# danbider/gp-quadrature

Hardware: AMD Instinct MI355X
Metric: GP-fits/sec (fit + posterior mean at the N training points), N=1e6 d=2 SE kernel (higher is better)
Workload: dtype f64; 1 GPU; 2D squared-exponential l=0.2 var=2 sigma2=0.2, eps=1e-4, global N=1e6 synthetic (BASELINE configs[1] at the metric's N=1e6), points sharded over the GPUs; n_per_gpu=1000000, global_n=1000000, d=2, mtot=23, M=529, mean_cg_iters=68, parallelism=points sharded over 1 GPU(s), CG replicated

## Files before the change

gp-quadrature_amd/csrc/nufft.hip:

```cpp
#include <cmath>
#include <cstdlib>
#include <cstring>
#include <optional>
#include <vector>

#include "common.hpp"
#include "es_kernel.hpp"
#include "nufft_dev.hpp"
#include "nufft_plan_host.hpp"
#include "points_layout.hpp"
#include "spread_mfma.hpp"
#include "small_dft.hpp"
#include "line_fft.hpp"

namespace efgp {


struct SpreadArgs {
    const double* x;
    StrengthSrc src;
    int64_t npts;
    GridGeom g;
    const double* coef;
    int degree;
// ... 1152 lines not shown
                    const double2 v = in ? f0[(int64_t)x0 * a.nf1 + x1] : make_double2(0.0, 0.0);
                    ire[u] = __double_as_longlong(v.x);
                    iim[u] = __double_as_longlong(v.y);
                } else {
                    ire[u] = in ? g0[(int64_t)x0 * a.nf1 + x1] : 0;
                    iim[u] = (in && a.channels == 2) ? g0[cells + (int64_t)x0 * a.nf1 + x1] : 0;
                }
            }
            if (r0 == 0) __syncthreads();
#pragma unroll
            for (int u = 0; u < U; ++u) {
                const double re = FINE ? __longlong_as_double(ire[u]) : (double)ire[u] * s0;
                const double im = FINE ? __longlong_as_double(iim[u]) : (double)iim[u] * s1;
#pragma unroll
                for (int jj = 0; jj < 2; ++jj) {
                    const double2 tw = T0[idx[jj]];
                    pq[jj].x += re * tw.x;
                    pq[jj].y += re * tw.y;
                    rs[jj].x += im * tw.x;
                    rs[jj].y += im * tw.y;
                    idx[jj] += step[jj];
                    if (idx[jj] >= a.nf0) idx[jj] -= a.nf0;
                }
            }
        }
#pragma unroll
        for (int jj = 0; jj < 2; ++jj) {
            Bp[grp][2 * jj][x1] = pq[jj];
            Bp[grp][2 * jj + 1][x1] = rs[jj];
        }
    }
    __syncthreads();
    unsigned int arrived = 0u;
    if (!FINE && tid == 0) arrived = atomicAdd(a.ticket, 1u);
    for (int o = tid; o < 2 * a.nf1; o += kG2MThreads) {
        const int jj = o / a.nf1, x = o - jj * a.nf1;
        double2 u = Bp[0][2 * jj][x], v = Bp[0][2 * jj + 1][x];
#pragma unroll
        for (int g = 1; g < kGroups; ++g) {
            u.x += Bp[g][2 * jj][x].x;
            u.y += Bp[g][2 * jj][x].y;
            v.x += Bp[g][2 * jj + 1][x].x;
            v.y += Bp[g][2 * jj + 1][x].y;
        }
        Bp[0][2 * jj][x] = make_double2(u.x - v.y, u.y + v.x);
        Bp[0][2 * jj + 1][x] = make_double2(u.x + v.y, v.x - u.y);
    }
    __syncthreads();
    if (nsplit > 1) {
        double2* const mine = a.partial + ((((int64_t)b * gridDim.x + blockIdx.x) * nsplit + split) * 4) * a.nf1;
        for (int o = tid; o < 4 * a.nf1; o += kG2MThreads) mine[o] = Bp[0][o / a.nf1][o % a.nf1];
        __threadfence();
        __syncthreads();
        if (tid == 0) {
            const unsigned int t = atomicAdd(a.tile_ticket + (int64_t)b * gridDim.x + blockIdx.x, 1u);
            s_last = (t == (unsigned)nsplit - 1u) ? 1 : 0;
        }
        __syncthreads();
        const bool tile_last = s_last != 0;
        __syncthreads();
        if (!tile_last) {
            if (tid == 0) s_last = (!FINE && arrived == a.total_wgs - 1u) ? 1 : 0;
            __syncthreads();
            if (s_last) {
                for (long long i = tid; i < a.acc_words; i += kG2MThreads) a.gacc[i] = 0;
                if (tid == 0) *a.ticket = 0u;
            }
            return;
        }
        __threadfence();
        const double2* const all = a.partial + (((int64_t)b * gridDim.x + blockIdx.x) * nsplit * 4) * a.nf1;
        for (int o = tid; o < 4 * a.nf1; o += kG2MThreads) {
            double2 u = all[o];
            for (int sp = 1; sp < nsplit; ++sp) {
                const double2 v = all[(int64_t)sp * 4 * a.nf1 + o];
                u.x += v.x;
                u.y += v.y;
            }
            Bp[0][o / a.nf1][o % a.nf1] = u;
        }
        if (tid == 0) a.tile_ticket[(int64_t)b * gridDim.x + blockIdx.x] = 0u;
        __syncthreads();
    }
    const int nk1 = 2 * a.h1 + 1;
    double2* const Hq = &Bp[1][0][0];
    for (int o = tid; o < 16 * nk1; o += kG2MThreads) {
        const int qtr = o / (4 * nk1), rc = o - qtr * 4 * nk1;
        const int r = rc / nk1, c = rc - r * nk1;
        int st = (c - a.h1) % a.nf1;
        if (st < 0) st += a.nf1;
        const int xa = (a.nf1 * qtr) / 4, xe = (a.nf1 * (qtr + 1)) / 4;
        int idx = (int)(((long long)st * xa) % a.nf1);
        double sx = 0.0, sy = 0.0;
        for (int x = xa; x < xe; ++x) {
            const double2 bv = Bp[0][r][x], tw = T1[idx];
            sx += bv.x * tw.x - bv.y * tw.y;
            sy += bv.x * tw.y + bv.y * tw.x;
            idx += st;
            if (idx >= a.nf1) idx -= a.nf1;
        }
        Hq[(qtr * 4 + r) * (2 * kG2MMaxH + 2) + c] = make_double2(sx, sy);
    }
    if (tid == 0) s_last = (!FINE && arrived == a.total_wgs - 1u) ? 1 : 0;
    __syncthreads();
    if (s_last) {
        for (long long i = tid; i < a.acc_words; i += kG2MThreads) a.gacc[i] = 0;
        if (tid == 0) *a.ticket = 0u;
    }
    for (int o = tid; o < 4 * nk1; o += kG2MThreads) {
        const int r = o / nk1, c = o - r * nk1;
        double2 u = Hq[r * (2 * kG2MMaxH + 2) + c];
#pragma unroll
        for (int q = 1; q < 4; ++q) {
            const double2 v = Hq[(q * 4 + r) * (2 * kG2MMaxH + 2) + c];
            u.x += v.x;
            u.y += v.y;
        }
        Hs[r][c] = u;
    }
    __syncthreads();
    for (int o = tid; o < 4 * nk1; o += kG2MThreads) {
        const int r = o / nk1, c = o - r * nk1;
        const int j = j0 + (r >> 1);
        if (j > a.h0 || (j == 0 && (r & 1))) continue;
        const int k0 = (r & 1) ? -j : j, k1 = c - a.h1;
        const double2 H = Hs[r][c], G = Hs[r ^ 1][nk1 - 1 - c];
        int64_t t;
        double f;
        if (a.part == 0) {
            if (g2m_slot(a.ma, k0, k1, &t, &f)) a.out_a[(int64_t)b * a.ma.total + t] = make_double2(H.x * f, H.y * f);
            continue;
        }
        if (g2m_slot(a.ma, k0, k1, &t, &f)) {
            double2 r1 = make_double2(0.5 * (H.x + G.x) * f, 0.5 * (H.y - G.y) * f);
            if (a.part == 3) {
                a.out_a[(int64_t)(2 * b) * a.ma.total + t] = r1;
                if (2 * b + 1 < a.rows_limit)
                    a.out_a[(int64_t)(2 * b + 1) * a.ma.total + t] = make_double2(0.5 * (H.y + G.y) * f, 0.5 * (G.x - H.x) * f);
            } else {
                const double norm0 = a.scale ? a.scale[4] : 1.0;
                if (norm0 != 1.0) {
                    r1.x *= norm0;
                    r1.y *= norm0;
                }
                a.out_a[t] = r1;
            }
        }
        if (a.part == 4 && g2m_slot(a.mb, k0, k1, &t, &f)) a.out_b[t] = make_double2(0.5 * (H.y + G.y) * f, 0.5 * (G.x - H.x) * f);
    }
}

constexpr int kG2RThreads = 1024;
constexpr int kR2MThreads = 256;

struct G2RArgs {
    long long* gacc;
    const double2* fine;
    const double* scale;
    int channels, nf0, nf1, h0, h1;
    int part, rows_limit, sign;
    ModeGeom ma, mb;
    double2* out_a;
    double2* out_b;
    double2* cbuf;
};

template <bool FINE>
__global__ __launch_bounds__(kG2RThreads) void grid_rows_kernel(G2RArgs a) {
    extern __shared__ double2 g2r_lds[];
    const int tid = threadIdx.x, b = blockIdx.y;
    const int nf0 = a.nf0, nf1 = a.nf1, h1 = a.h1;
    const int nk1 = 2 * h1 + 1;
    const int64_t cells = (int64_t)nf0 * nf1;
    double2* const T = g2r_lds;
    double2* const Row = T + 256;
    for (int q = tid; q < nf1; q += kG2RThreads) {
        double sn, cs;
        sincospi((double)a.sign * 2.0 * (double)q / (double)nf1, &sn, &cs);
        T[q] = make_double2(cs, sn);
    }
    const int x0_lo = (int)blockIdx.x * kG2RRows;
    {
        const double s0 = FINE ? 1.0 : a.scale[1], s1 = FINE ? 1.0 : a.scale[3];
        for (int o = tid; o < kG2RRows * nf1; o += kG2RThreads) {
            const int r = o / nf1, x1 = o - r * nf1, x0 = x0_lo + r;
            double2 v = make_double2(0.0, 0.0);
            if (x0 < nf0) {
                if (FINE) {
                    v = a.fine[(int64_t)b * cells + (int64_t)x0 * nf1 + x1];
                } else {
                    long long* g = a.gacc + (int64_t)b * a.channels * cells + (int64_t)x0 * nf1 + x1;
                    const long long ire = g[0];
                    g[0] = 0;
                    long long iim = 0;
                    if (a.channels == 2) {
                        iim = g[cells];
                        g[cells] = 0;
                    }
                    v = make_double2((double)ire * s0, (double)iim * s1);
                }
            }
            Row[o] = v;
        }
    }
    __syncthreads();
    constexpr int SEG = 8;
    const int seg = tid & (SEG - 1), pair = tid >> 3;
    const int npairs = kG2RRows * (h1 + 1);
    for (int pr = pair; pr < ((npairs + 127) / 128) * 128; pr += 128) {
        const bool on = pr < npairs;
        const int r = on ? pr / (h1 + 1) : 0, k1 = on ? pr - r * (h1 + 1) : 0;
        const int xa = (nf1 * seg) / SEG, xe = (nf1 * (seg + 1)) / SEG;
        int idx = (int)(((long long)k1 * xa) % nf1);
        double P = 0.0, Q = 0.0, R = 0.0, S = 0.0;
        if (on) {
            const double2* row = Row + r * nf1;
            for (int x = xa; x < xe; ++x) {
                const double2 g = row[x], tw = T[idx];
                P = fma(g.x, tw.x, P);
                Q = fma(g.x, tw.y, Q);
                R = fma(g.y, tw.x, R);
                S = fma(g.y, tw.y, S);
                idx += k1;
                if (idx >= nf1) idx -= nf1;
            }
        }
#pragma unroll
        for (int m = 1; m < SEG; m <<= 1) {
            P += __shfl_xor(P, m, 64);
            Q += __shfl_xor(Q, m, 64);
            R += __shfl_xor(R, m, 64);
            S += __shfl_xor(S, m, 64);
        }
        const int x0 = x0_lo + r;
        if (on && seg == 0 && x0 < nf0) {
            double2* c = a.cbuf + ((int64_t)b * nf0 + x0) * nk1;
            c[h1 + k1] = make_double2(P - S, Q + R);
            if (k1 > 0) c[h1 - k1] = make_double2(P + S, R - Q);
        }
    }
}

__global__ __launch_bounds__(kR2MThreads) void rows_modes_kernel(G2RArgs a) {
    __shared__ double2 T[256], Cc[2][256], Hs[2][2 * kG2MMaxH + 2], part[2][4][2 * kG2MMaxH + 2];
    const int tid = threadIdx.x, b = blockIdx.y, k1 = (int)blockIdx.x;
    const int nf0 = a.nf0, h0 = a.h0, h1 = a.h1;
    const int nk0 = 2 * h0 + 1, nk1 = 2 * h1 + 1;
    const double2* C = a.cbuf + (int64_t)b * nf0 * nk1;
    for (int o = tid; o < 2 * nf0; o += kR2MThreads) {
        const int col = o >= nf0 ? 1 : 0, x0 = o - col * nf0;
        Cc[col][x0] = C[(int64_t)x0 * nk1 + (col ? h1 - k1 : h1 + k1)];
    }
    for (int q = tid; q < nf0; q += kR2MThreads) {
        double sn, cs;
        sincospi((double)a.sign * 2.0 * (double)q / (double)nf0, &sn, &cs);
        T[q] = make_double2(cs, sn);
    }
    __syncthreads();
    for (int o = tid; o < 8 * nk0; o += kR2MThreads) {
        const int qtr = o / (2 * nk0), rc = o - qtr * 2 * nk0;
        const int col = rc / nk0, r = rc - col * nk0;
        int st = (r - h0) % nf0;
        if (st < 0) st += nf0;
        const int xa = (nf0 * qtr) / 4, xe = (nf0 * (qtr + 1)) / 4;
        int idx = (int)(((long long)st * xa) % nf0);
        double sx = 0.0, sy = 0.0;
        for (int x = xa; x < xe; ++x) {
            const double2 cv = Cc[col][x], tw = T[idx];
            sx = fma(cv.x, tw.x, fma(-cv.y, tw.y, sx));
            sy = fma(cv.x, tw.y, fma(cv.y, tw.x, sy));
            idx += st;
            if (idx >= nf0) idx -= nf0;
        }
        part[col][qtr][r] = make_double2(sx, sy);
    }
    __syncthreads();
    for (int o = tid; o < 2 * nk0; o += kR2MThreads) {
        const int col = o / nk0, r = o - col * nk0;
        Hs[col][r] = make_double2((part[col][0][r].x + part[col][1][r].x) + (part[col][2][r].x + part[col][3][r].x),
                                  (part[col][0][r].y + part[col][1][r].y) + (part[col][2][r].y + part[col][3][r].y));
    }
    __syncthreads();
    for (int o = tid; o < 2 * nk0; o += kR2MThreads) {
        const int col = o / nk0, r = o - col * nk0;
        if (col == 1 && k1 == 0) continue;
        const int k0 = r - h0, kk1 = col ? -k1 : k1;
        const double2 H = Hs[col][r], G = Hs[k1 == 0 ? 0 : 1 - col][nk0 - 1 - r];
        int64_t t;
        double f;
        if (a.part == 0) {
            if (g2m_slot(a.ma, k0, kk1, &t, &f)) a.out_a[(int64_t)b * a.ma.total + t] = make_double2(H.x * f, H.y * f);
            continue;
        }
        if (g2m_slot(a.ma, k0, kk1, &t, &f)) {
            double2 r1 = make_double2(0.5 * (H.x + G.x) * f, 0.5 * (H.y - G.y) * f);
            if (a.part == 3) {
                a.out_a[(int64_t)(2 * b) * a.ma.total + t] = r1;
                if (2 * b + 1 < a.rows_limit)
                    a.out_a[(int64_t)(2 * b + 1) * a.ma.total + t] = make_double2(0.5 * (H.y + G.y) * f, 0.5 * (G.x - H.x) * f);
            } else {
                const double norm0 = a.scale ? a.scale[4] : 1.0;
                if (norm0 != 1.0) {
                    r1.x *= norm0;
                    r1.y *= norm0;
                }
                a.out_a[t] = r1;
            }
        }
        if (a.part == 4 && g2m_slot(a.mb, k0, kk1, &t, &f)) a.out_b[t] = make_double2(0.5 * (H.y + G.y) * f, 0.5 * (G.x - H.x) * f);
    }
}

__global__ void precorrect_kernel(const double2* __restrict__ fin, const double2* __restrict__ mul, ModeGeom m, int herm,
                                  int64_t cells, double2* __restrict__ fine) {
    const int batch = blockIdx.y;
    const double2* fb = fin + (int64_t)batch * m.total;
    double2* F = fine + (int64_t)batch * cells;
    for (int64_t c = (int64_t)blockIdx.x * blockDim.x + threadIdx.x; c < cells; c += (int64_t)gridDim.x * blockDim.x) {
        int64_t rem = c;
        int64_t ks[3] = {0, 0, 0};
        bool inside = true;
        for (int a = m.d - 1; a >= 0; --a) {
            const int64_t i = rem % m.nf[a];
            rem /= m.nf[a];
            const int64_t k = i <= (m.nf[a] - 1) / 2 ? i : i - m.nf[a];
            ks[a] = k;
            inside = inside && k >= -(m.nm[a] / 2) && k <= (m.nm[a] - 1) / 2;
        }
        double2 r = make_double2(0.0, 0.0);
        if (inside) {
            int64_t t = 0, tn = 0;
            bool has_neg = true;
            double f = 1.0;
            for (int a = 0; a < m.d; ++a) {
                const int64_t k = ks[a], kmin = -(m.nm[a] / 2), kmax = (m.nm[a] - 1) / 2;
                f *= m.fac[a][k - kmin];
                t = t * m.nm[a] + (m.modeord == 0 ? k - kmin : (k >= 0 ? k : k + m.nm[a]));
                const int64_t kn = -k;
                if (kn < kmin || kn > kmax) has_neg = false;
                tn = tn * m.nm[a] + (m.modeord == 0 ? kn - kmin : (kn >= 0 ? kn : kn + m.nm[a]));
            }
            double2 v = fb[t];
            if (mul) v = make_double2(v.x * mul[t].x - v.y * mul[t].y, v.x * mul[t].y + v.y * mul[t].x);
            if (herm && has_neg) {
                double2 u = fb[tn];
                if (mul) u = make_double2(u.x * mul[tn].x - u.y * mul[tn].y, u.x * mul[tn].y + u.y * mul[tn].x);
                v = make_double2(0.5 * (v.x + u.x), 0.5 * (v.y - u.y));
            }
            r = make_double2(v.x * f, v.y * f);
        }
        F[c] = r;
    }
}

struct InterpArgs {
    const double* x;
    int64_t npts;
    GridGeom g;
    const double* coef;
    int degree;
    const double2* fine;
    void* out;
    const int* order;
    const double* image;
};

template <int D, int W, bool CPLX, bool USE_LDS>
__global__ __launch_bounds__(USE_LDS ? kInterpThreads : kInterpThreadsGlobal) void interp_kernel(InterpArgs a) {
    constexpr int kThr = USE_LDS ? kInterpThreads : kInterpThreadsGlobal;
    extern __shared__ double lds[];
    const int batch = blockIdx.y;
    const int64_t cells = a.g.cells;
    const double2* F = a.fine + (int64_t)batch * cells;
    if (USE_LDS) {
        if (CPLX) {
            double2* l2 = reinterpret_cast<double2*>(lds);
            for (int64_t i = threadIdx.x; i < cells; i += kThr) l2[i] = F[i];
        } else {
            for (int64_t i = threadIdx.x; i < cells; i += kThr) lds[i] = F[i].x;
        }
        __syncthreads();
    }
    const int nf0 = (int)a.g.nf[0], nf1 = (int)a.g.nf[1], nf2 = (int)a.g.nf[2];
    auto load = [&](int64_t i, double& re, double& im) {
        if (USE_LDS) {
            if (CPLX) {
                double2 v = reinterpret_cast<const double2*>(lds)[i];
                re = v.x;
                im = v.y;
            } else {
                re = lds[i];
                im = 0.0;
            }
        } else {
            if (CPLX) {
                double2 v = F[i];
                re = v.x;
                im = v.y;
            } else {
                re = F[i].x;
                im = 0.0;
            }
        }
    };
    for (int64_t n = (int64_t)blockIdx.x * kThr + threadIdx.x; n < a.npts;
         n += (int64_t)gridDim.x * kThr) {
        double v0[W], v1[W], v2[W];
        int f0 = 0, f1 = 0, f2 = 0;
        {
            double Xw[3] = {0.0, 0.0, 0.0};
            Xw[0] = fold(a.g.scale[0] * (a.x[n * D + 0] - a.g.xcen[0]), (double)nf0);
            if (D > 1) Xw[1] = fold(a.g.scale[1] * (a.x[n * D + 1] - a.g.xcen[1]), (double)nf1);
            if (D > 2) Xw[2] = fold(a.g.scale[2] * (a.x[n * D + 2] - a.g.xcen[2]), (double)nf2);
            window_eval<D, W>(a.coef, a.degree, Xw, nf0, nf1, nf2, f0, f1, f2, v0, v1, v2);
        }
        double sre = 0.0, sim = 0.0;
        if (D == 1) {
#pragma unroll
            for (int j = 0; j < W; ++j) {
                double re, im;
                load(wrap(f0 + j, nf0), re, im);
                sre = fma(v0[j], re, sre);
                if (CPLX) sim = fma(v0[j], im, sim);
            }
        } else if (D == 2) {
#pragma unroll
            for (int j0 = 0; j0 < W; ++j0) {
                const int row = wrap(f0 + j0, nf0) * nf1;
                double rre = 0.0, rim = 0.0;
#pragma unroll
                for (int j1 = 0; j1 < W; ++j1) {
                    double re, im;
                    load(row + wrap(f1 + j1, nf1), re, im);
                    rre = fma(v1[j1], re, rre);
                    if (CPLX) rim = fma(v1[j1], im, rim);
                }
                sre = fma(v0[j0], rre, sre);
                if (CPLX) sim = fma(v0[j0], rim, sim);
            }
        } else {
// ... 684 lines not shown
    int* hist = tmp;
    int* cursor = tmp + t.nbins + 1;
    KernelTimer* order_timer = new KernelTimer("order", stream);
    EFGP_HIP_CHECK(hipMemsetAsync(hist, 0, (size_t)(t.nbins + 1) * sizeof(int), stream));
    const int nwg = (int)std::max<int64_t>(1, (plan->npts + 32 * 1024 - 1) / (32 * 1024));
    const size_t lds_h = (size_t)t.nbins * sizeof(int), lds_s = (size_t)2 * t.nbins * sizeof(int);
#define EFGP_BIN_LAUNCH(D_)                                                                                              \
    if (lds_s > 65536) {                                                                                                  \
        EFGP_HIP_CHECK(hipFuncSetAttribute((const void*)bin_scatter_kernel<D_>, hipFuncAttributeMaxDynamicSharedMemorySize, \
                                           (int)lds_s));                                                                  \
    }                                                                                                                     \
    if (lds_h > 65536) {                                                                                                  \
        EFGP_HIP_CHECK(hipFuncSetAttribute((const void*)bin_hist_kernel<D_>, hipFuncAttributeMaxDynamicSharedMemorySize,  \
                                           (int)lds_h));                                                                  \
    }                                                                                                                     \
    hipLaunchKernelGGL((bin_hist_kernel<D_>), dim3(nwg), dim3(1024), lds_h, stream, t, plan->x, plan->npts, hist);        \
    hipLaunchKernelGGL(bin_scan_kernel, dim3(1), dim3(1024), 0, stream, (const int*)hist, t.nbins, b->start, cursor);     \
    hipLaunchKernelGGL((bin_scatter_kernel<D_>), dim3(nwg), dim3(1024), lds_s, stream, t, plan->x, plan->npts, cursor,    \
                       b->xs, b->order);
    if (plan->dim == 1) { EFGP_BIN_LAUNCH(1) }
    else if (plan->dim == 2) { EFGP_BIN_LAUNCH(2) }
    else { EFGP_BIN_LAUNCH(3) }
#undef EFGP_BIN_LAUNCH
    delete order_timer;
    EFGP_HIP_CHECK(hipGetLastError());
    if (plan->dim == 3) {
        int rcb = balance_tiles(plan, b, stream);
        if (rcb != EFGP_OK) return rcb;
    }
    plan->bins.push_back(b);
    *out = b;
    return EFGP_OK;
}

template <int D>
static hipError_t launch_tile_d(int W, dim3 grid, size_t lds_bytes, hipStream_t s, const TileSpreadArgs& a) {
    switch (W) {
#define EFGP_CASE(w_)                                                                                               \
    case w_: {                                                                                                      \
        auto k = strength_is_normal(a.src.mode) ? spread_tile_kernel<D, w_, true> : spread_tile_kernel<D, w_, false>; \
        if (lds_bytes > 65536) {                                                                                    \
            hipError_t e = hipFuncSetAttribute((const void*)k, hipFuncAttributeMaxDynamicSharedMemorySize, (int)lds_bytes); \
            if (e != hipSuccess) return e;                                                                          \
        }                                                                                                           \
        hipLaunchKernelGGL(k, grid, dim3(kSpreadThreads), lds_bytes, s, a);                                         \
        return hipGetLastError();                                                                                   \
    }
        EFGP_CASE(2) EFGP_CASE(3) EFGP_CASE(4) EFGP_CASE(5) EFGP_CASE(6) EFGP_CASE(7) EFGP_CASE(8) EFGP_CASE(9)
        EFGP_CASE(10) EFGP_CASE(11) EFGP_CASE(12) EFGP_CASE(13) EFGP_CASE(14) EFGP_CASE(15) EFGP_CASE(16)
#undef EFGP_CASE
    }
    return hipErrorInvalidValue;
}

template <int W>
static hipError_t launch_cell_w(int channels, int degree, dim3 grid, hipStream_t s, const CellSpreadArgs& a) {
    if (degree <= W + 2) {
        if (channels == 2) hipLaunchKernelGGL((spread_cell_kernel<W, 2, W + 2>), grid, dim3(256), kCellLds, s, a);
        else hipLaunchKernelGGL((spread_cell_kernel<W, 1, W + 2>), grid, dim3(256), kCellLds, s, a);
    } else {
        if (channels == 2) hipLaunchKernelGGL((spread_cell_kernel<W, 2, W + 4>), grid, dim3(256), kCellLds, s, a);
        else hipLaunchKernelGGL((spread_cell_kernel<W, 1, W + 4>), grid, dim3(256), kCellLds, s, a);
    }
    return hipGetLastError();
}
static hipError_t launch_cell(int W, int channels, int degree, dim3 grid, hipStream_t s, const CellSpreadArgs& a) {
    switch (W) {
#define EFGP_CASE(w_) case w_: return launch_cell_w<w_>(channels, degree, grid, s, a);
        EFGP_CASE(2) EFGP_CASE(3) EFGP_CASE(4) EFGP_CASE(5) EFGP_CASE(6) EFGP_CASE(7) EFGP_CASE(8)
#undef EFGP_CASE
    }
    return hipErrorInvalidValue;
}

static char* scale_slot(DeviceCtx* ctx, hipStream_t stream) {
    char* misc = (char*)scratch(ctx, SLOT_SCALE, 64);
    if (misc && !ctx->scale_slot_ready) {
        if (hipMemsetAsync(misc, 0, 64, stream) != hipSuccess) return nullptr;
        ctx->scale_slot_ready = true;
    }
    return misc;
}

struct G2MRequest {
    int part = 0;
    int rows_limit = 1 << 30;
    ModeGeom ma, mb;
    void* out_a = nullptr;
    void* out_b = nullptr;
    bool done = false;
    bool cropped = false;
    int64_t crop_nf[3] = {1, 1, 1};
};
static void apply_crop(const G2MRequest* req, ModeGeom& m, int64_t& cells) {
    if (!req || !req->cropped) return;
    cells = 1;
    for (int a = 0; a < 3; ++a) {
        if (a < m.d) m.nf[a] = req->crop_nf[a];
        cells *= a < m.d ? req->crop_nf[a] : 1;
    }
}

static ModeBoxes mode_boxes(const G2MRequest& req) {
    ModeBoxes b;
    b.part = req.part;
    for (int a = 0; a < 3; ++a) {
        b.nma[a] = req.ma.nm[a];
        b.nmb[a] = req.part == 4 ? req.mb.nm[a] : 1;
    }
    return b;
}

static int g2m_launch(DeviceCtx* ctx, const Type1Plan& pl, const GridGeom& g, G2MRequest* req, long long* gacc, const double2* fine,
                      const double* scale, int channels, int nbatch, int isign, unsigned int* ticket, long long acc_words,
                      hipStream_t stream) {
    G2MArgs ga;
    ga.gacc = gacc;
    ga.fine = fine;
    ga.scale = scale;
    ga.channels = channels;
    ga.nf0 = (int)g.nf[0];
    ga.nf1 = (int)g.nf[1];
    ga.h0 = pl.g2m_h[0];
    ga.h1 = pl.g2m_h[1];
    ga.part = req->part;
    ga.rows_limit = req->rows_limit;
    ga.sign = isign < 0 ? -1 : 1;
    ga.ma = req->ma;
    ga.mb = req->part == 4 ? req->mb : req->ma;
    ga.out_a = (double2*)req->out_a;
    ga.out_b = (double2*)req->out_b;
    ga.ticket = ticket;
    if (pl.g2m_two_launch) {
        G2RArgs ra;
        ra.gacc = gacc;
        ra.fine = fine;
        ra.scale = scale;
        ra.channels = channels;
        ra.nf0 = ga.nf0;
        ra.nf1 = ga.nf1;
        ra.h0 = ga.h0;
        ra.h1 = ga.h1;
        ra.part = ga.part;
        ra.rows_limit = ga.rows_limit;
        ra.sign = ga.sign;
        ra.ma = ga.ma;
        ra.mb = ga.mb;
        ra.out_a = ga.out_a;
        ra.out_b = ga.out_b;
        const int nk1 = 2 * ga.h1 + 1;
        ra.cbuf = (double2*)scratch(ctx, SLOT_G2M, (size_t)nbatch * ga.nf0 * nk1 * sizeof(double2));
        if (!ra.cbuf) return EFGP_ENOMEM;
        ctx->g2m_zeroed_for = nullptr;
        const size_t lds = (256 + (size_t)kG2RRows * ga.nf1) * sizeof(double2);
        const dim3 grid((ga.nf0 + kG2RRows - 1) / kG2RRows, nbatch);
        if (gacc) hipLaunchKernelGGL((grid_rows_kernel<false>), grid, dim3(kG2RThreads), lds, stream, ra);
        else hipLaunchKernelGGL((grid_rows_kernel<true>), grid, dim3(kG2RThreads), lds, stream, ra);
        EFGP_HIP_CHECK(hipGetLastError());
        hipLaunchKernelGGL(rows_modes_kernel, dim3(ga.h1 + 1, nbatch), dim3(kR2MThreads), 0, stream, ra);
        EFGP_HIP_CHECK(hipGetLastError());
        req->done = true;
        return EFGP_OK;
    }
    const unsigned tiles = (unsigned)(ga.h0 / 2 + 1);
    const bool small = ga.nf0 <= 128 && ga.nf1 <= 128;
    const int split = pl.g2m_split;
    constexpr size_t kTicketBytes = 65536;
    ga.partial = nullptr;
    ga.tile_ticket = nullptr;
    if (split > 1) {
        const size_t bytes = kTicketBytes + (size_t)nbatch * tiles * split * 4 * ga.nf1 * sizeof(double2);
        char* base = (char*)scratch(ctx, SLOT_G2M, bytes);
        if (!base) return EFGP_ENOMEM;
        if (ctx->g2m_zeroed_for != (const void*)base) {
            EFGP_HIP_CHECK(hipMemsetAsync(base, 0, kTicketBytes, stream));
            ctx->g2m_zeroed_for = base;
        }
        ga.tile_ticket = (unsigned int*)base;
        ga.partial = (double2*)(base + kTicketBytes);
    }
    ga.total_wgs = tiles * (unsigned)nbatch * (unsigned)split;
    ga.acc_words = acc_words;
    const dim3 grid(tiles, nbatch, split);
    if (gacc && small) hipLaunchKernelGGL((grid_to_modes_kernel<false, 7>), grid, dim3(kG2MThreads), 0, stream, ga);
    else if (gacc) hipLaunchKernelGGL((grid_to_modes_kernel<false, 8>), grid, dim3(kG2MThreads), 0, stream, ga);
    else if (small) hipLaunchKernelGGL((grid_to_modes_kernel<true, 7>), grid, dim3(kG2MThreads), 0, stream, ga);
    else hipLaunchKernelGGL((grid_to_modes_kernel<true, 8>), grid, dim3(kG2MThreads), 0, stream, ga);
    EFGP_HIP_CHECK(hipGetLastError());
    req->done = true;
    return EFGP_OK;
}

static int transform_fine(efgp_nufft_s* plan, const Type1Plan& pl, const GridGeom& g, double2* fine, int nbatch, int isign, hipStream_t stream,
                          G2MRequest* req, const double* scale, double2** fine_out, const FftAccSource* acc = nullptr) {
    auto convert = [&]() -> int {
        if (!acc) return EFGP_OK;
        const int rb = (int)((g.cells + 63) / 64);
        hipLaunchKernelGGL((reduce_slabs_kernel<true>), dim3(rb, nbatch), dim3(512), 0, stream, (const double*)acc->acc, 1, acc->channels,
                           g.cells, acc->scale, fine, acc->reset);
        EFGP_HIP_CHECK(hipGetLastError());
        return EFGP_OK;
    };
    int rcc = EFGP_OK;
    switch (pl.after) {
        case AfterSpread::g2m_from_acc:
        case AfterSpread::g2m:
            if ((rcc = convert()) != EFGP_OK) return rcc;
            *fine_out = nullptr;
            return g2m_launch(plan->ctx, pl, g, req, nullptr, fine, scale, 2, nbatch, isign, nullptr, 0, stream);
        case AfterSpread::pruned_from_acc:
        case AfterSpread::pruned: {
            double2* work = (double2*)scratch(plan->ctx, SLOT_FFT_WORK, (size_t)pl.work_cells * sizeof(double2));
            if (!work) return EFGP_ENOMEM;
            double2* res = nullptr;
            const bool fuse = pl.after == AfterSpread::pruned_from_acc;
            if (!fuse && (rcc = convert()) != EFGP_OK) return rcc;
            const int rcp = own_fft_pruned_forward(plan->ctx, plan->dim, g.nf, pl.nc, nbatch, fine, work, isign < 0, &res, stream, fuse ? acc : nullptr);
            if (rcp != EFGP_OK) return rcp;
            req->cropped = true;
            for (int a = 0; a < 3; ++a) req->crop_nf[a] = pl.nc[a];
            *fine_out = res;
            return EFGP_OK;
        }
        case AfterSpread::fft: break;
    }
    if ((rcc = convert()) != EFGP_OK) return rcc;
    const int rc = fft_c2c(plan->ctx, plan->dim, g.nf, nbatch, fine, isign < 0, stream);
    if (rc != EFGP_OK) return rc;
    *fine_out = fine;
    return EFGP_OK;
}

struct SpreadJob {
    StrengthSrc src;
    int channels;
    bool need_max;
    double floor_bound;
    const double* max_src;
    double max_mult;
    int64_t nvals;
    int ones_channel;
};

static SpreadJob make_spread_job(int mode, const double* c, const double* point_scale, int nbatch, int64_t npts,
                                 unsigned long long seed = 0, int64_t index_offset = 0) {
    const bool normal = strength_is_normal(mode);
    const bool scaled = point_scale != nullptr && normal;
    const bool from_memory = mode == STR_REAL || mode == STR_COMPLEX || mode == STR_REAL_AND_ONES || mode == STR_REAL_PAIR;
    const bool two_channels = mode == STR_COMPLEX || mode == STR_REAL_AND_ONES || mode == STR_REAL_PAIR || mode == STR_RNG_PAIR ||
                              mode == STR_NORMAL_PAIR;
    const bool unit = mode == STR_REAL_AND_ONES || mode == STR_ONES || mode == STR_RNG || mode == STR_RNG_PAIR;
    const bool two_per_point = mode == STR_COMPLEX || mode == STR_REAL_PAIR;
    SpreadJob j;
    j.src = StrengthSrc{c, npts, mode, seed, index_offset, scaled ? point_scale : nullptr};
    j.channels = two_channels ? 2 : 1;
    j.need_max = from_memory || scaled;
    j.floor_bound = scaled ? 0.0 : normal ? kNormalBound : unit ? 1.0 : 0.0;
    j.max_src = scaled ? point_scale : c;
    j.max_mult = scaled ? kNormalBound : 1.0;
    j.nvals = (mode == STR_REAL_AND_ONES || scaled) ? npts : (int64_t)nbatch * npts * (two_per_point ? 2 : 1);
    j.ones_channel = mode == STR_REAL_AND_ONES ? 1 : 0;
    return j;
}

static ScaleJob scale_job(const SpreadJob& job, int64_t per, int sum_bits, double* scale) {
    return ScaleJob{job.floor_bound, job.ones_channel, per, scale, sum_bits, job.max_mult};
}

static void enqueue_scale(const SpreadJob& job, const ScaleJob& sj, char* misc, hipStream_t stream) {
    if (job.need_max) {
        const int blocks = (int)std::max<int64_t>(1, std::min<int64_t>((job.nvals + 8191) / 8192, 256));
        hipLaunchKernelGGL(maxabs_kernel, dim3(blocks), dim3(1024), 0, stream, job.max_src, job.nvals, (unsigned long long*)(misc + 56),
                           (unsigned int*)(misc + 48), sj);
    } else {
        hipLaunchKernelGGL(fixed_scale_kernel, dim3(1), dim3(64), 0, stream, sj.floor_bound, sj.ones_channel, sj.per, sj.scale,
                           sj.sum_bits);
    }
}

template <class F>
static inline hipError_t by_dim(int dim, F&& f) {
    if (dim == 1) return f(std::integral_constant<int, 1>{});
    if (dim == 2) return f(std::integral_constant<int, 2>{});
    return f(std::integral_constant<int, 3>{});
}

static int get_class_order(efgp_nufft_s* plan, const WindowSet* w, const GridGeom& g, int nwg, int64_t per, hipStream_t stream,
                           const int** out) {
    ClassOrder* co = nullptr;
    for (ClassOrder* o : plan->orders)
        if (o->W == w->p.w && o->nwg == nwg && o->nf[0] == g.nf[0] && o->nf[1] == g.nf[1] && o->nf[2] == g.nf[2]) co = o;
    if (!co) {
        co = new ClassOrder();
        for (int q = 0; q < 3; ++q) co->nf[q] = g.nf[q];
        co->W = w->p.w;
        co->nwg = nwg;
        co->bytes = (size_t)plan->npts * sizeof(int);
        co->order = (int*)pool_alloc(plan->ctx, co->bytes);
        if (!co->order) {
            delete co;
            return EFGP_ENOMEM;
        }
        const unsigned blocks = nwg > 0 ? (unsigned)nwg : (unsigned)((plan->npts + kOrderWindow - 1) / kOrderWindow);
        if (nwg == 0) per = kOrderWindow;
        KernelTimer order_timer("order", stream);
        if (plan->dim == 2)
            hipLaunchKernelGGL((class_order_kernel<2, 16>), dim3(blocks), dim3(kSpreadThreads), 0, stream, g, w->p.w, plan->x, plan->npts, per,
                               co->order);
        else
            hipLaunchKernelGGL((class_order_kernel<3, 16>), dim3(blocks), dim3(kSpreadThreads), 0, stream, g, w->p.w, plan->x, plan->npts, per,
                               co->order);
        EFGP_HIP_CHECK(hipGetLastError());
// ... 719 lines not shown
```

gp-quadrature_amd/csrc/small_dft.hip:

```cpp
#include "small_dft.hpp"

#include "nufft_plan_host.hpp"

#include <algorithm>

namespace efgp {

constexpr int kDftThreads = 256;

struct M2GArgs {
    const double2* f;
    const double2* mul;
    int nm0, nm1, modeord, isign;
    const double *fac0, *fac1;
    int nf0, nf1;
    double2* fine;
    double* image;
    int p0, p1;
};

__global__ __launch_bounds__(kDftThreads) void modes_to_grid_real_kernel(M2GArgs a) {
    __shared__ double2 tw0[kDftMaxNf], tw1[kDftMaxNf], t[64], part[4][64];
    extern __shared__ double2 cm[];
    const int nf0 = a.nf0, nf1 = a.nf1, nm0 = a.nm0, nm1 = a.nm1;
    const double sgn = a.isign < 0 ? -2.0 : 2.0;
    for (int i = threadIdx.x; i < nf0; i += kDftThreads) {
        double s, c;
        sincospi(sgn * (double)i / (double)nf0, &s, &c);
        tw0[i] = make_double2(c, s);
    }
    for (int i = threadIdx.x; i < nf1; i += kDftThreads) {
        double s, c;
        sincospi(sgn * (double)i / (double)nf1, &s, &c);
        tw1[i] = make_double2(c, s);
    }
    for (int i = threadIdx.x; i < nm0 * nm1; i += kDftThreads) {
        const int s0 = i / nm1, s1 = i - s0 * nm1;
        const int k0 = s0 - nm0 / 2, k1 = s1 - nm1 / 2;
        const int slot0 = a.modeord == 0 ? s0 : (k0 >= 0 ? k0 : k0 + nm0);
        const int slot1 = a.modeord == 0 ? s1 : (k1 >= 0 ? k1 : k1 + nm1);
        const int64_t idx = (int64_t)slot0 * nm1 + slot1;
        double2 v = a.f[idx];
        if (a.mul) {
            const double2 m = a.mul[idx];
            v = make_double2(v.x * m.x - v.y * m.y, v.x * m.y + v.y * m.x);
        }
        const double fc = a.fac0[s0] * a.fac1[s1];
        cm[i] = make_double2(v.x * fc, v.y * fc);
    }
    __syncthreads();
    const int x0 = blockIdx.x;
    {
        const int s1 = threadIdx.x & 63, qtr = threadIdx.x >> 6;
        if (s1 < nm1) {
            const int lo = (nm0 * qtr) / 4, hi = (nm0 * (qtr + 1)) / 4;
            int ph = (int)(((int64_t)(lo - nm0 / 2) * x0) % nf0);
            ph = ph < 0 ? ph + nf0 : ph;
            double re = 0.0, im = 0.0;
            for (int s0 = lo; s0 < hi; ++s0) {
                const double2 v = cm[s0 * nm1 + s1], w = tw0[ph];
                re += v.x * w.x - v.y * w.y;
                im += v.x * w.y + v.y * w.x;
                ph += x0;
                ph = ph >= nf0 ? ph - nf0 : ph;
            }
            part[qtr][s1] = make_double2(re, im);
        }
    }
    __syncthreads();
    if ((int)threadIdx.x < nm1) {
        const int s1 = threadIdx.x;
        t[s1] = make_double2(part[0][s1].x + part[1][s1].x + part[2][s1].x + part[3][s1].x,
                             part[0][s1].y + part[1][s1].y + part[2][s1].y + part[3][s1].y);
    }
    __syncthreads();
    for (int x1 = threadIdx.x; x1 < nf1; x1 += kDftThreads) {
        int ph = (int)(((int64_t)(-(nm1 / 2)) * x1) % nf1);
        ph = ph < 0 ? ph + nf1 : ph;
        double re = 0.0;
        for (int s1 = 0; s1 < nm1; ++s1) {
            re += t[s1].x * tw1[ph].x - t[s1].y * tw1[ph].y;
            ph += x1;
            ph = ph >= nf1 ? ph - nf1 : ph;
        }
        if (a.image == nullptr) {
            a.fine[(int64_t)x0 * nf1 + x1] = make_double2(re, 0.0);
            continue;
        }
        const int p1 = a.p1, plane = a.p0 * p1;
        for (int r = x0; r < a.p0; r += nf0) {
            double* row = a.image + r * p1;
            for (int c = x1; c < p1; c += nf1) row[c] = re;
            for (int c = x1 == 0 ? nf1 - 1 : x1 - 1; c < p1; c += nf1) row[plane + c] = re;
        }
    }
}


int modes_to_grid_real_launch(DeviceCtx* ctx, const double2* f, const double2* mul, int nm0, int nm1, int modeord, int isign,
                              const double* fac0, const double* fac1, int nf0, int nf1, double2* fine, double* image, int p0, int p1,
                              hipStream_t stream) {
    (void)ctx;
    M2GArgs a{f, mul, nm0, nm1, modeord, isign, fac0, fac1, nf0, nf1, fine, image, p0, p1};
    const size_t lds = (size_t)nm0 * nm1 * sizeof(double2);
    if (lds > 32 * 1024) EFGP_HIP_CHECK(hipFuncSetAttribute((const void*)modes_to_grid_real_kernel, hipFuncAttributeMaxDynamicSharedMemorySize, (int)lds));
    hipLaunchKernelGGL(modes_to_grid_real_kernel, dim3(nf0), dim3(kDftThreads), lds, stream, a);
    EFGP_HIP_CHECK(hipGetLastError());
    return EFGP_OK;
}

}
```

Baseline: 4345 GP fits/s of the global N=1e6 problem (whole job; the points are sharded over the GPUs).

## Batch LDS loads in small-DFT kernels and overlap twiddle setup with global loads

Restructures the small direct-DFT kernels (grid-to-rows, rows-to-modes, modes-to-grid) so that each inner loop loads groups of eight values and twiddles before doing the FMAs, with a sched barrier between the two phases. This hides LDS latency. It also skews the LDS layout to avoid bank conflicts, widens rows_modes to 512 threads so one thread loads one value, and folds the quarter reduction into the output pass, dropping one barrier. Global loads are issued before the twiddle sincospi so the two overlap, and the image replication writes are spread over thread slices. The old serial path stays available behind an environment variable, at the cost of extra code and template variants.

Measured after the change: 4460 GP fits/s of the global N=1e6 problem (whole job; the points are sharded over the GPUs), median of 6. 1.03x the previous value.

```diff
diff --git a/gp-quadrature_amd/csrc/nufft.hip b/gp-quadrature_amd/csrc/nufft.hip
--- a/gp-quadrature_amd/csrc/nufft.hip
+++ b/gp-quadrature_amd/csrc/nufft.hip
@@ -1328,6 +1328,7 @@
 
 constexpr int kG2RThreads = 1024;
 constexpr int kR2MThreads = 256;
+constexpr int kR2MThreadsWide = 512;
 
 struct G2RArgs {
     long long* gacc;
@@ -1341,7 +1342,44 @@
     double2* cbuf;
 };
 
-template <bool FINE>
+__device__ __forceinline__ void g2r_acc(double& P, double& Q, double& R, double& S, const double2 g, const double2 tw) {
+    P = fma(g.x, tw.x, P);
+    Q = fma(g.x, tw.y, Q);
+    R = fma(g.y, tw.x, R);
+    S = fma(g.y, tw.y, S);
+}
+__device__ __forceinline__ void r2m_acc(double& sx, double& sy, const double2 cv, const double2 tw) {
+    sx = fma(cv.x, tw.x, fma(-cv.y, tw.y, sx));
+    sy = fma(cv.x, tw.y, fma(cv.y, tw.x, sy));
+}
+constexpr int kDftGroup = 8;
+__host__ __device__ __forceinline__ constexpr int dft_skew(int i) { return i + (i >> 4); }
+constexpr int kDftSkewTable = dft_skew(256);
+template <bool FULL, bool SKEW, typename Acc>
+__device__ __forceinline__ void dft_group(const double2* __restrict__ v, const double2* __restrict__ T, int x, int n, int& idx,
+                                          int step, int nf, Acc acc) {
+    double2 g[kDftGroup], tw[kDftGroup];
+#pragma unroll
+    for (int j = 0; j < kDftGroup; ++j) {
+        const int xx = x + (FULL ? j : min(j, n - 1));
+        g[j] = v[SKEW ? dft_skew(xx) : xx];
+        tw[j] = T[SKEW ? dft_skew(idx) : idx];
+        idx += step;
+        if (idx >= nf) idx -= nf;
+    }
+    __builtin_amdgcn_sched_barrier(0);
+#pragma unroll
+    for (int j = 0; j < kDftGroup; ++j)
+        if (FULL || j == 0 || j < n) acc(g[j], tw[j]);
+}
+
+static_assert(kG2RRows * kG2MMaxNf <= kG2RThreads, "one accumulator cell per thread");
+__host__ __device__ __forceinline__ constexpr int g2r_row_pitch(int nf1) { return dft_skew(nf1) + 1; }
+static size_t g2r_lds_bytes(int nf1, bool serial) {
+    return serial ? (256 + (size_t)kG2RRows * nf1) * sizeof(double2)
+                  : ((size_t)kDftSkewTable + (size_t)kG2RRows * g2r_row_pitch(nf1)) * sizeof(double2);
+}
+template <bool FINE, bool SERIAL>
 __global__ __launch_bounds__(kG2RThreads) void grid_rows_kernel(G2RArgs a) {
     extern __shared__ double2 g2r_lds[];
     const int tid = threadIdx.x, b = blockIdx.y;
@@ -1349,14 +1387,43 @@
     const int nk1 = 2 * h1 + 1;
     const int64_t cells = (int64_t)nf0 * nf1;
     double2* const T = g2r_lds;
-    double2* const Row = T + 256;
-    for (int q = tid; q < nf1; q += kG2RThreads) {
-        double sn, cs;
-        sincospi((double)a.sign * 2.0 * (double)q / (double)nf1, &sn, &cs);
-        T[q] = make_double2(cs, sn);
-    }
+    double2* const Row = T + (SERIAL ? 256 : kDftSkewTable);
+    const int row_pitch = SERIAL ? nf1 : g2r_row_pitch(nf1);
     const int x0_lo = (int)blockIdx.x * kG2RRows;
-    {
+    if constexpr (!SERIAL) {
+        const double s0 = FINE ? 1.0 : a.scale[1], s1 = FINE ? 1.0 : a.scale[3];
+        const int o = tid;
+        const int r = o / nf1, x1 = o - r * nf1, x0 = x0_lo + r;
+        const bool cell = o < kG2RRows * nf1, live = cell && x0 < nf0;
+        double2 v = make_double2(0.0, 0.0);
+        long long ire = 0, iim = 0;
+        if (live) {
+            if (FINE) {
+                v = a.fine[(int64_t)b * cells + (int64_t)x0 * nf1 + x1];
+            } else {
+                long long* g = a.gacc + (int64_t)b * a.channels * cells + (int64_t)x0 * nf1 + x1;
+                ire = g[0];
+                if (a.channels == 2) iim = g[cells];
+                g[0] = 0;
+                if (a.channels == 2) g[cells] = 0;
+            }
+        }
+        const int q = kG2RRows * nf1 <= kG2RThreads / 2 ? tid - kG2RThreads / 2 : tid;
+        if (q >= 0 && q < nf1) {
+            double sn, cs;
+            sincospi((double)a.sign * 2.0 * (double)q / (double)nf1, &sn, &cs);
+            T[dft_skew(q)] = make_double2(cs, sn);
+        }
+        if (FINE) asm volatile("" : "+v"(v.x), "+v"(v.y));
+        else asm volatile("" : "+v"(ire), "+v"(iim));
+        if (!FINE && live) v = make_double2((double)ire * s0, (double)iim * s1);
+        if (cell) Row[r * row_pitch + dft_skew(x1)] = v;
+    } else {
+        for (int q = tid; q < nf1; q += kG2RThreads) {
+            double sn, cs;
+            sincospi((double)a.sign * 2.0 * (double)q / (double)nf1, &sn, &cs);
+            T[q] = make_double2(cs, sn);
+        }
         const double s0 = FINE ? 1.0 : a.scale[1], s1 = FINE ? 1.0 : a.scale[3];
         for (int o = tid; o < kG2RRows * nf1; o += kG2RThreads) {
             const int r = o / nf1, x1 = o - r * nf1, x0 = x0_lo + r;
@@ -1390,15 +1457,19 @@
         int idx = (int)(((long long)k1 * xa) % nf1);
         double P = 0.0, Q = 0.0, R = 0.0, S = 0.0;
         if (on) {
-            const double2* row = Row + r * nf1;
-            for (int x = xa; x < xe; ++x) {
-                const double2 g = row[x], tw = T[idx];
-                P = fma(g.x, tw.x, P);
-                Q = fma(g.x, tw.y, Q);
-                R = fma(g.y, tw.x, R);
-                S = fma(g.y, tw.y, S);
-                idx += k1;
-                if (idx >= nf1) idx -= nf1;
+            const double2* row = Row + r * row_pitch;
+            if constexpr (SERIAL) {
+                for (int x = xa; x < xe; ++x) {
+                    const double2 g = row[x], tw = T[idx];
+                    g2r_acc(P, Q, R, S, g, tw);
+                    idx += k1;
+                    if (idx >= nf1) idx -= nf1;
+                }
+            } else {
+                const auto acc = [&](const double2 g, const double2 tw) { g2r_acc(P, Q, R, S, g, tw); };
+                int x = xa;
+                for (; x + kDftGroup <= xe; x += kDftGroup) dft_group<true, true>(row, T, x, kDftGroup, idx, k1, nf1, acc);
+                if (x < xe) dft_group<false, true>(row, T, x, xe - x, idx, k1, nf1, acc);
             }
         }
 #pragma unroll
@@ -1417,23 +1488,43 @@
     }
 }
 
-__global__ __launch_bounds__(kR2MThreads) void rows_modes_kernel(G2RArgs a) {
-    __shared__ double2 T[256], Cc[2][256], Hs[2][2 * kG2MMaxH + 2], part[2][4][2 * kG2MMaxH + 2];
+__device__ __forceinline__ double2 r2m_quarters(const double2 (*p)[2 * kG2MMaxH + 2], int r) {
+    return make_double2((p[0][r].x + p[1][r].x) + (p[2][r].x + p[3][r].x), (p[0][r].y + p[1][r].y) + (p[2][r].y + p[3][r].y));
+}
+
+static_assert(2 * kG2MMaxNf <= kR2MThreadsWide, "one value of C per thread");
+template <bool SERIAL>
+__global__ __launch_bounds__(SERIAL ? kR2MThreads : kR2MThreadsWide) void rows_modes_kernel(G2RArgs a) {
+    constexpr int NT = SERIAL ? kR2MThreads : kR2MThreadsWide;
+    __shared__ double2 T[256], Cc[2][256], part[2][4][2 * kG2MMaxH + 2];
     const int tid = threadIdx.x, b = blockIdx.y, k1 = (int)blockIdx.x;
     const int nf0 = a.nf0, h0 = a.h0, h1 = a.h1;
     const int nk0 = 2 * h0 + 1, nk1 = 2 * h1 + 1;
     const double2* C = a.cbuf + (int64_t)b * nf0 * nk1;
-    for (int o = tid; o < 2 * nf0; o += kR2MThreads) {
-        const int col = o >= nf0 ? 1 : 0, x0 = o - col * nf0;
-        Cc[col][x0] = C[(int64_t)x0 * nk1 + (col ? h1 - k1 : h1 + k1)];
-    }
-    for (int q = tid; q < nf0; q += kR2MThreads) {
-        double sn, cs;
-        sincospi((double)a.sign * 2.0 * (double)q / (double)nf0, &sn, &cs);
-        T[q] = make_double2(cs, sn);
+    if constexpr (SERIAL) {
+        for (int o = tid; o < 2 * nf0; o += NT) {
+            const int col = o >= nf0 ? 1 : 0, x0 = o - col * nf0;
+            Cc[col][x0] = C[(int64_t)x0 * nk1 + (col ? h1 - k1 : h1 + k1)];
+        }
+        for (int q = tid; q < nf0; q += NT) {
+            double sn, cs;
+            sincospi((double)a.sign * 2.0 * (double)q / (double)nf0, &sn, &cs);
+            T[q] = make_double2(cs, sn);
+        }
+    } else {
+        const int col = tid >= nf0 ? 1 : 0, x0 = tid - col * nf0;
+        const bool ld = tid < 2 * nf0;
+        double2 cv = make_double2(0.0, 0.0);
+        if (ld) cv = C[(int64_t)x0 * nk1 + (col ? h1 - k1 : h1 + k1)];
+        if (tid < nf0) {
+            double sn, cs;
+            sincospi((double)a.sign * 2.0 * (double)tid / (double)nf0, &sn, &cs);
+            T[tid] = make_double2(cs, sn);
+        }
+        if (ld) Cc[col][x0] = cv;
     }
     __syncthreads();
-    for (int o = tid; o < 8 * nk0; o += kR2MThreads) {
+    for (int o = tid; o < 8 * nk0; o += NT) {
         const int qtr = o / (2 * nk0), rc = o - qtr * 2 * nk0;
         const int col = rc / nk0, r = rc - col * nk0;
         int st = (r - h0) % nf0;
@@ -1441,27 +1532,37 @@
         const int xa = (nf0 * qtr) / 4, xe = (nf0 * (qtr + 1)) / 4;
         int idx = (int)(((long long)st * xa) % nf0);
         double sx = 0.0, sy = 0.0;
-        for (int x = xa; x < xe; ++x) {
-            const double2 cv = Cc[col][x], tw = T[idx];
-            sx = fma(cv.x, tw.x, fma(-cv.y, tw.y, sx));
-            sy = fma(cv.x, tw.y, fma(cv.y, tw.x, sy));
-            idx += st;
-            if (idx >= nf0) idx -= nf0;
+        if constexpr (SERIAL) {
+            for (int x = xa; x < xe; ++x) {
+                const double2 cv = Cc[col][x], tw = T[idx];
+                r2m_acc(sx, sy, cv, tw);
+                idx += st;
+                if (idx >= nf0) idx -= nf0;
+            }
+        } else {
+            const auto acc = [&](const double2 cv, const double2 tw) { r2m_acc(sx, sy, cv, tw); };
+            int x = xa;
+            for (; x + kDftGroup <= xe; x += kDftGroup) dft_group<true, false>(Cc[col], T, x, kDftGroup, idx, st, nf0, acc);
+            if (x < xe) dft_group<false, false>(Cc[col], T, x, xe - x, idx, st, nf0, acc);
         }
         part[col][qtr][r] = make_double2(sx, sy);
     }
     __syncthreads();
-    for (int o = tid; o < 2 * nk0; o += kR2MThreads) {
-        const int col = o / nk0, r = o - col * nk0;
-        Hs[col][r] = make_double2((part[col][0][r].x + part[col][1][r].x) + (part[col][2][r].x + part[col][3][r].x),
-                                  (part[col][0][r].y + part[col][1][r].y) + (part[col][2][r].y + part[col][3][r].y));
-    }
-    __syncthreads();
-    for (int o = tid; o < 2 * nk0; o += kR2MThreads) {
+    __shared__ double2 Hs[2][2 * kG2MMaxH + 2];
+    if constexpr (SERIAL) {
+        for (int o = tid; o < 2 * nk0; o += NT) {
+            const int col = o / nk0, r = o - col * nk0;
+            Hs[col][r] = r2m_quarters(part[col], r);
+        }
+        __syncthreads();
+    }
+    for (int o = tid; o < 2 * nk0; o += NT) {
         const int col = o / nk0, r = o - col * nk0;
         if (col == 1 && k1 == 0) continue;
         const int k0 = r - h0, kk1 = col ? -k1 : k1;
-        const double2 H = Hs[col][r], G = Hs[k1 == 0 ? 0 : 1 - col][nk0 - 1 - r];
+        const int gcol = k1 == 0 ? 0 : 1 - col, gr = nk0 - 1 - r;
+        const double2 H = SERIAL ? Hs[col][r] : r2m_quarters(part[col], r);
+        const double2 G = SERIAL ? Hs[gcol][gr] : r2m_quarters(part[gcol], gr);
         int64_t t;
         double f;
         if (a.part == 0) {
@@ -2452,12 +2553,16 @@
         ra.cbuf = (double2*)scratch(ctx, SLOT_G2M, (size_t)nbatch * ga.nf0 * nk1 * sizeof(double2));
         if (!ra.cbuf) return EFGP_ENOMEM;
         ctx->g2m_zeroed_for = nullptr;
-        const size_t lds = (256 + (size_t)kG2RRows * ga.nf1) * sizeof(double2);
         const dim3 grid((ga.nf0 + kG2RRows - 1) / kG2RRows, nbatch);
-        if (gacc) hipLaunchKernelGGL((grid_rows_kernel<false>), grid, dim3(kG2RThreads), lds, stream, ra);
-        else hipLaunchKernelGGL((grid_rows_kernel<true>), grid, dim3(kG2RThreads), lds, stream, ra);
+        const bool serial = std::getenv("EFGP_SMALL_DFT_SERIAL") != nullptr;
+        const size_t lds = g2r_lds_bytes(ga.nf1, serial);
+        if (gacc && serial) hipLaunchKernelGGL((grid_rows_kernel<false, true>), grid, dim3(kG2RThreads), lds, stream, ra);
+        else if (gacc) hipLaunchKernelGGL((grid_rows_kernel<false, false>), grid, dim3(kG2RThreads), lds, stream, ra);
+        else if (serial) hipLaunchKernelGGL((grid_rows_kernel<true, true>), grid, dim3(kG2RThreads), lds, stream, ra);
+        else hipLaunchKernelGGL((grid_rows_kernel<true, false>), grid, dim3(kG2RThreads), lds, stream, ra);
         EFGP_HIP_CHECK(hipGetLastError());
-        hipLaunchKernelGGL(rows_modes_kernel, dim3(ga.h1 + 1, nbatch), dim3(kR2MThreads), 0, stream, ra);
+        if (serial) hipLaunchKernelGGL(rows_modes_kernel<true>, dim3(ga.h1 + 1, nbatch), dim3(kR2MThreads), 0, stream, ra);
+        else hipLaunchKernelGGL(rows_modes_kernel<false>, dim3(ga.h1 + 1, nbatch), dim3(kR2MThreadsWide), 0, stream, ra);
         EFGP_HIP_CHECK(hipGetLastError());
         req->done = true;
         return EFGP_OK;
diff --git a/gp-quadrature_amd/csrc/small_dft.hip b/gp-quadrature_amd/csrc/small_dft.hip
--- a/gp-quadrature_amd/csrc/small_dft.hip
+++ b/gp-quadrature_amd/csrc/small_dft.hip
@@ -3,6 +3,7 @@
 #include "nufft_plan_host.hpp"
 
 #include <algorithm>
+#include <cstdlib>
 
 namespace efgp {
 
@@ -19,34 +20,89 @@
     int p0, p1;
 };
 
+__device__ __forceinline__ double m2g_re(double ax, double ay, double bx, double by) { return fma(ax, bx, -(ay * by)); }
+__device__ __forceinline__ double m2g_im(double ax, double ay, double bx, double by) { return fma(ay, bx, ax * by); }
+__device__ __forceinline__ double2 m2g_cmul(double2 v, double2 m) {
+    return make_double2(m2g_re(v.x, v.y, m.x, m.y), m2g_im(v.x, v.y, m.x, m.y));
+}
+__device__ __forceinline__ double2 m2g_scale(double2 v, double f0, double f1) {
+    const double fc = f0 * f1;
+    return make_double2(v.x * fc, v.y * fc);
+}
+__device__ __forceinline__ void m2g_acc(double& re, double& im, double2 v, double2 w) {
+    re += m2g_re(v.x, v.y, w.x, w.y);
+    im += m2g_im(v.x, v.y, w.x, w.y);
+}
+
+constexpr int kDftGroup = 8;
+constexpr int kDftLoadTrips = 4;
+static_assert(2 * kDftMaxNf <= kDftThreads, "one twiddle per thread");
+
+template <bool SERIAL>
 __global__ __launch_bounds__(kDftThreads) void modes_to_grid_real_kernel(M2GArgs a) {
     __shared__ double2 tw0[kDftMaxNf], tw1[kDftMaxNf], t[64], part[4][64];
+    __shared__ double res[kDftMaxNf];
     extern __shared__ double2 cm[];
     const int nf0 = a.nf0, nf1 = a.nf1, nm0 = a.nm0, nm1 = a.nm1;
     const double sgn = a.isign < 0 ? -2.0 : 2.0;
-    for (int i = threadIdx.x; i < nf0; i += kDftThreads) {
-        double s, c;
-        sincospi(sgn * (double)i / (double)nf0, &s, &c);
-        tw0[i] = make_double2(c, s);
-    }
-    for (int i = threadIdx.x; i < nf1; i += kDftThreads) {
-        double s, c;
-        sincospi(sgn * (double)i / (double)nf1, &s, &c);
-        tw1[i] = make_double2(c, s);
-    }
-    for (int i = threadIdx.x; i < nm0 * nm1; i += kDftThreads) {
-        const int s0 = i / nm1, s1 = i - s0 * nm1;
-        const int k0 = s0 - nm0 / 2, k1 = s1 - nm1 / 2;
-        const int slot0 = a.modeord == 0 ? s0 : (k0 >= 0 ? k0 : k0 + nm0);
-        const int slot1 = a.modeord == 0 ? s1 : (k1 >= 0 ? k1 : k1 + nm1);
-        const int64_t idx = (int64_t)slot0 * nm1 + slot1;
-        double2 v = a.f[idx];
-        if (a.mul) {
-            const double2 m = a.mul[idx];
-            v = make_double2(v.x * m.x - v.y * m.y, v.x * m.y + v.y * m.x);
-        }
-        const double fc = a.fac0[s0] * a.fac1[s1];
-        cm[i] = make_double2(v.x * fc, v.y * fc);
+    if constexpr (SERIAL) {
+        for (int i = threadIdx.x; i < nf0; i += kDftThreads) {
+            double s, c;
+            sincospi(sgn * (double)i / (double)nf0, &s, &c);
+            tw0[i] = make_double2(c, s);
+        }
+        for (int i = threadIdx.x; i < nf1; i += kDftThreads) {
+            double s, c;
+            sincospi(sgn * (double)i / (double)nf1, &s, &c);
+            tw1[i] = make_double2(c, s);
+        }
+        for (int i = threadIdx.x; i < nm0 * nm1; i += kDftThreads) {
+            const int s0 = i / nm1, s1 = i - s0 * nm1;
+            const int k0 = s0 - nm0 / 2, k1 = s1 - nm1 / 2;
+            const int slot0 = a.modeord == 0 ? s0 : (k0 >= 0 ? k0 : k0 + nm0);
+            const int slot1 = a.modeord == 0 ? s1 : (k1 >= 0 ? k1 : k1 + nm1);
+            const int64_t idx = (int64_t)slot0 * nm1 + slot1;
+            double2 v = a.f[idx];
+            if (a.mul) v = m2g_cmul(v, a.mul[idx]);
+            cm[i] = m2g_scale(v, a.fac0[s0], a.fac1[s1]);
+        }
+    } else {
+        const int nmodes = nm0 * nm1;
+        const bool has_mul = a.mul != nullptr;
+        bool tables = false;
+        for (int base = threadIdx.x; base < nmodes || !tables; base += kDftLoadTrips * kDftThreads) {
+            double2 v[kDftLoadTrips], m[kDftLoadTrips];
+            double f0[kDftLoadTrips], f1[kDftLoadTrips];
+#pragma unroll
+            for (int j = 0; j < kDftLoadTrips; ++j) {
+                const int i = min(base + j * kDftThreads, nmodes - 1);
+                const int s0 = i / nm1, s1 = i - s0 * nm1;
+                const int k0 = s0 - nm0 / 2, k1 = s1 - nm1 / 2;
+                const int slot0 = a.modeord == 0 ? s0 : (k0 >= 0 ? k0 : k0 + nm0);
+                const int slot1 = a.modeord == 0 ? s1 : (k1 >= 0 ? k1 : k1 + nm1);
+                const int64_t idx = (int64_t)slot0 * nm1 + slot1;
+                v[j] = a.f[idx];
+                m[j] = has_mul ? a.mul[idx] : make_double2(0.0, 0.0);
+                f0[j] = a.fac0[s0];
+                f1[j] = a.fac1[s1];
+            }
+            if (!tables) {
+                const int i = threadIdx.x;
+                const bool first = i < nf0;
+                const int q = first ? i : i - nf0, n = first ? nf0 : nf1;
+                if (q < n) {
+                    double s, c;
+                    sincospi(sgn * (double)q / (double)n, &s, &c);
+                    (first ? tw0 : tw1)[q] = make_double2(c, s);
+                }
+                tables = true;
+            }
+#pragma unroll
+            for (int j = 0; j < kDftLoadTrips; ++j) {
+                const int i = base + j * kDftThreads;
+                if (i < nmodes) cm[i] = m2g_scale(has_mul ? m2g_cmul(v[j], m[j]) : v[j], f0[j], f1[j]);
+            }
+        }
     }
     __syncthreads();
     const int x0 = blockIdx.x;
@@ -57,12 +113,29 @@
             int ph = (int)(((int64_t)(lo - nm0 / 2) * x0) % nf0);
             ph = ph < 0 ? ph + nf0 : ph;
             double re = 0.0, im = 0.0;
-            for (int s0 = lo; s0 < hi; ++s0) {
-                const double2 v = cm[s0 * nm1 + s1], w = tw0[ph];
-                re += v.x * w.x - v.y * w.y;
-                im += v.x * w.y + v.y * w.x;
-                ph += x0;
-                ph = ph >= nf0 ? ph - nf0 : ph;
+            if constexpr (SERIAL) {
+                for (int s0 = lo; s0 < hi; ++s0) {
+                    const double2 v = cm[s0 * nm1 + s1], w = tw0[ph];
+                    m2g_acc(re, im, v, w);
+                    ph += x0;
+                    ph = ph >= nf0 ? ph - nf0 : ph;
+                }
+            } else {
+                for (int g0 = lo; g0 < hi; g0 += kDftGroup) {
+                    const int n = min(kDftGroup, hi - g0);
+                    double2 v[kDftGroup], w[kDftGroup];
+#pragma unroll
+                    for (int j = 0; j < kDftGroup; ++j) {
+                        v[j] = cm[(g0 + min(j, n - 1)) * nm1 + s1];
+                        w[j] = tw0[ph];
+                        ph += x0;
+                        ph = ph >= nf0 ? ph - nf0 : ph;
+                    }
+                    __builtin_amdgcn_sched_barrier(0);
+#pragma unroll
+                    for (int j = 0; j < kDftGroup; ++j)
+                        if (j == 0 || j < n) m2g_acc(re, im, v[j], w[j]);
+                }
             }
             part[qtr][s1] = make_double2(re, im);
         }
@@ -74,24 +147,68 @@
                              part[0][s1].y + part[1][s1].y + part[2][s1].y + part[3][s1].y);
     }
     __syncthreads();
-    for (int x1 = threadIdx.x; x1 < nf1; x1 += kDftThreads) {
-        int ph = (int)(((int64_t)(-(nm1 / 2)) * x1) % nf1);
-        ph = ph < 0 ? ph + nf1 : ph;
-        double re = 0.0;
-        for (int s1 = 0; s1 < nm1; ++s1) {
-            re += t[s1].x * tw1[ph].x - t[s1].y * tw1[ph].y;
-            ph += x1;
-            ph = ph >= nf1 ? ph - nf1 : ph;
-        }
-        if (a.image == nullptr) {
-            a.fine[(int64_t)x0 * nf1 + x1] = make_double2(re, 0.0);
-            continue;
-        }
+    if constexpr (SERIAL) {
+        for (int x1 = threadIdx.x; x1 < nf1; x1 += kDftThreads) {
+            int ph = (int)(((int64_t)(-(nm1 / 2)) * x1) % nf1);
+            ph = ph < 0 ? ph + nf1 : ph;
+            double re = 0.0;
+            for (int s1 = 0; s1 < nm1; ++s1) {
+                re += m2g_re(t[s1].x, t[s1].y, tw1[ph].x, tw1[ph].y);
+                ph += x1;
+                ph = ph >= nf1 ? ph - nf1 : ph;
+            }
+            if (a.image == nullptr) {
+                a.fine[(int64_t)x0 * nf1 + x1] = make_double2(re, 0.0);
+                continue;
+            }
+            const int p1 = a.p1, plane = a.p0 * p1;
+            for (int r = x0; r < a.p0; r += nf0) {
+                double* row = a.image + r * p1;
+                for (int c = x1; c < p1; c += nf1) row[c] = re;
+                for (int c = x1 == 0 ? nf1 - 1 : x1 - 1; c < p1; c += nf1) row[plane + c] = re;
+            }
+        }
+    } else {
+        const int x1 = threadIdx.x;
+        if (x1 < nf1) {
+            int ph = (int)(((int64_t)(-(nm1 / 2)) * x1) % nf1);
+            ph = ph < 0 ? ph + nf1 : ph;
+            double re = 0.0;
+            for (int g0 = 0; g0 < nm1; g0 += kDftGroup) {
+                const int n = min(kDftGroup, nm1 - g0);
+                double2 v[kDftGroup], w[kDftGroup];
+#pragma unroll
+                for (int j = 0; j < kDftGroup; ++j) {
+                    v[j] = t[g0 + min(j, n - 1)];
+                    w[j] = tw1[ph];
+                    ph += x1;
+                    ph = ph >= nf1 ? ph - nf1 : ph;
+                }
+                __builtin_amdgcn_sched_barrier(0);
+#pragma unroll
+                for (int j = 0; j < kDftGroup; ++j)
+                    if (j == 0 || j < n) re += m2g_re(v[j].x, v[j].y, w[j].x, w[j].y);
+            }
+            if (a.image == nullptr) a.fine[(int64_t)x0 * nf1 + x1] = make_double2(re, 0.0);
+            else res[x1] = re;
+        }
+        if (a.image == nullptr) return;
+        __syncthreads();
+        const int nsl = kDftThreads / nf1, sl = (int)threadIdx.x / nf1, c0 = (int)threadIdx.x - sl * nf1;
+        if (sl >= nsl) return;
+        const double re = res[c0];
         const int p1 = a.p1, plane = a.p0 * p1;
+        int turn = sl;
         for (int r = x0; r < a.p0; r += nf0) {
             double* row = a.image + r * p1;
-            for (int c = x1; c < p1; c += nf1) row[c] = re;
-            for (int c = x1 == 0 ? nf1 - 1 : x1 - 1; c < p1; c += nf1) row[plane + c] = re;
+            for (int c = c0; c < p1; c += nf1) {
+                if (turn == 0) row[c] = re;
+                turn = turn == 0 ? nsl - 1 : turn - 1;
+            }
+            for (int c = c0 == 0 ? nf1 - 1 : c0 - 1; c < p1; c += nf1) {
+                if (turn == 0) row[plane + c] = re;
+                turn = turn == 0 ? nsl - 1 : turn - 1;
+            }
         }
     }
 }
@@ -103,8 +220,11 @@
     (void)ctx;
     M2GArgs a{f, mul, nm0, nm1, modeord, isign, fac0, fac1, nf0, nf1, fine, image, p0, p1};
     const size_t lds = (size_t)nm0 * nm1 * sizeof(double2);
-    if (lds > 32 * 1024) EFGP_HIP_CHECK(hipFuncSetAttribute((const void*)modes_to_grid_real_kernel, hipFuncAttributeMaxDynamicSharedMemorySize, (int)lds));
-    hipLaunchKernelGGL(modes_to_grid_real_kernel, dim3(nf0), dim3(kDftThreads), lds, stream, a);
+    const bool serial = std::getenv("EFGP_SMALL_DFT_SERIAL") != nullptr;
+    const void* fn = serial ? (const void*)modes_to_grid_real_kernel<true> : (const void*)modes_to_grid_real_kernel<false>;
+    if (lds > 32 * 1024) EFGP_HIP_CHECK(hipFuncSetAttribute(fn, hipFuncAttributeMaxDynamicSharedMemorySize, (int)lds));
+    if (serial) hipLaunchKernelGGL(modes_to_grid_real_kernel<true>, dim3(nf0), dim3(kDftThreads), lds, stream, a);
+    else hipLaunchKernelGGL(modes_to_grid_real_kernel<false>, dim3(nf0), dim3(kDftThreads), lds, stream, a);
     EFGP_HIP_CHECK(hipGetLastError());
     return EFGP_OK;
 }
```
